# tuannv-github/srsRAN_Project

Hardware: AMD Instinct MI355X
Metric: PDSCH+PUSCH codeblocks/s @ 100 MHz 273-PRB 4x4 MIMO (PDSCH 4 layers, PUSCH 4 layers x 4 rx) (higher is better)
Workload: dtype int8+fp32; 1 GPU; BASELINE metric (PDSCH+PUSCH codeblocks/s @ 100 MHz 273-PRB 4x4 MIMO): full PDSCH+PUSCH slot pipeline, 100 MHz numerology-1 273 PRB, 256QAM R=948/1024; parallelism=single GPU

## Files before the change

### srsran_project_amd/csrc/pdsch_modulator.hip

```cpp
#include <hip/hip_runtime.h>

#include "bf16_device.h"

#include "gold_sequence.h"
#include "pdsch_modulator_args.h"

#pragma clang fp contract(off)

namespace srs_amd {
namespace {

__device__ __forceinline__ float2 cmul_simd(float2 x, float wr, float wi)
{
  return make_float2(__builtin_fmaf(x.x, wr, -(x.y * wi)), __builtin_fmaf(x.y, wr, x.x * wi));
}

__device__ __forceinline__ uint32_t to_bf16(float f)
{
  uint32_t u = __float_as_uint(f);
  u += 0x7fffu + ((u >> 16) & 1u);
  return u >> 16;
}

__device__ __forceinline__ uint32_t pack_cbf16(float2 v)
{
  return cbf16_pack(v.x, v.y);
}

__device__ __forceinline__ float2 qam_point(uint32_t idx, int qm)
{
  float off = -1.0f, re = 0.0f, im = 0.0f;
  for (int j = 0; j < qm / 2; ++j) {
    re += off;
    im += off;
    off *= 2.0f;
    re = ((idx >> (2 * j + 1)) & 1u) ? re : -re;
    im = ((idx >> (2 * j)) & 1u) ? im : -im;
  }
  return make_float2(re, im);
}

__device__ __forceinline__ uint32_t data_re_before(const uint32_t* row, uint32_t nof_prb, uint32_t k)
{
  const uint32_t prb = k / PDSCH_NRE;
  if (prb >= nof_prb) {
    const uint32_t e = row[nof_prb - 1];
    return (e >> 12) + __builtin_popcount(e & 0xfffu);
  }
  const uint32_t e = row[prb];
  return (e >> 12) + __builtin_popcount(e & ((1u << (k % PDSCH_NRE)) - 1u));
}

__device__ __forceinline__ uint32_t codeword_word(const uint8_t* cw, uint32_t nof_bytes, uint32_t w)
{
  uint32_t v = 0;
#pragma unroll
  for (int q = 0; q < 4; ++q) {
    const uint32_t p = 4 * w + q;
    const uint32_t b = p < nof_bytes ? cw[p] : 0u;
    v |= (__builtin_bitreverse32(b) >> 24) << (8 * q);
  }
  return v;
}

constexpr int MAX_WORDS = PDSCH_THREADS + 2;

template <bool MULTI, typename T>
__device__ __forceinline__ const T& item_of(const T& own, const T* items)
{
  if constexpr (MULTI) {
    return items[blockIdx.z];
  } else {
    return own;
  }
}

template <bool MULTI>
__global__ __launch_bounds__(PDSCH_THREADS) void pdsch_map_kernel(pdsch_map_args own, const pdsch_map_args* items)
{
  const pdsch_map_args& a = item_of<MULTI>(own, items);
  if (MULTI && (blockIdx.x >= a.nof_tiles || blockIdx.y >= a.nof_symbols)) {
    return;
  }
  __shared__ uint32_t scrambled[MAX_WORDS];
  __shared__ float2   s_qam[256];

  const uint32_t  l   = a.first_symbol + blockIdx.y;
  const uint32_t  k0  = a.first_subc + blockIdx.x * PDSCH_THREADS;
  const uint32_t  k   = k0 + threadIdx.x;
  const uint32_t* row = a.re_table + l * a.nof_prb;
  const uint32_t  kend = min(k0 + PDSCH_THREADS, a.nof_subc);

  const uint32_t bits_per_re = static_cast<uint32_t>(a.nof_layers) * (a.qm < 2 ? 1u : static_cast<uint32_t>(a.qm));
  const uint32_t j_lo        = data_re_before(row, a.nof_prb, k0);
  const uint32_t j_hi        = data_re_before(row, a.nof_prb, kend);
  if (j_hi == j_lo) {
    return;
  }
  const uint32_t w_lo = j_lo * bits_per_re / 32;
  const uint32_t w_hi = (j_hi * bits_per_re + 31) / 32;

  const uint8_t* cw        = a.codewords + static_cast<uint64_t>(blockIdx.z) * a.cw_stride;
  const uint32_t nof_bytes = (a.nof_bits + 7) / 8;
  if (a.qm >= 2 && threadIdx.x < (1u << a.qm)) {
    s_qam[threadIdx.x] = qam_point(threadIdx.x, a.qm);
  }
  const uint32_t nw = w_hi - w_lo;
  for (uint32_t q = threadIdx.x; q < nw; q += PDSCH_THREADS) {
    scrambled[q] = codeword_word(cw, nof_bytes, w_lo + q) ^ a.scr[w_lo + q];
  }
  __syncthreads();

  if (k >= kend) {
    return;
  }
  const uint32_t e   = row[k / PDSCH_NRE];
  const uint32_t bit = k % PDSCH_NRE;
  if (((e >> bit) & 1u) == 0) {
    return;
  }
  const uint32_t j = (e >> 12) + __builtin_popcount(e & ((1u << bit) - 1u));
  if ((j + 1) * bits_per_re > a.nof_bits) {
    return;
  }

  const int bps = a.qm < 2 ? 1 : a.qm;
  float2    x[4];
#pragma unroll
  for (int v = 0; v < 4; ++v) {
    if (v < a.nof_layers) {
      const uint32_t s   = j * a.nof_layers + v;
      const uint32_t o   = s * bps - w_lo * 32;
      const uint64_t win = static_cast<uint64_t>(scrambled[o / 32]) |
                           (static_cast<uint64_t>(scrambled[min(o / 32 + 1, static_cast<uint32_t>(MAX_WORDS - 1))])
                            << 32);
      const uint32_t seq = static_cast<uint32_t>(win >> (o % 32)) & ((1u << bps) - 1u);
      const uint32_t idx = __builtin_bitreverse32(seq) >> (32 - bps);
      if (a.qm >= 2) {
        x[v] = s_qam[idx];
      } else {
        const float b = idx ? -1.0f : 1.0f;
        x[v]          = make_float2((a.qm == 0 && (s & 1u)) ? -b : b, b);
      }
    }
  }

  uint32_t* grid = a.grids + static_cast<uint64_t>(blockIdx.z) * a.grid_stride + l * a.nof_subc + k;
#pragma unroll
  for (int p = 0; p < 4; ++p) {
    if (p < a.nof_ports) {
      float2 y = cmul_simd(x[0], a.w[0][p][0], a.w[0][p][1]);
#pragma unroll
      for (int v = 1; v < 4; ++v) {
        if (v < a.nof_layers) {
          const float2 t = cmul_simd(x[v], a.w[v][p][0], a.w[v][p][1]);
          y.x            = y.x + t.x;
          y.y            = y.y + t.y;
        }
      }
      grid[static_cast<uint64_t>(p) * a.port_stride] = pack_cbf16(y);
    }
  }
}

constexpr int DMRS_THREADS      = 256;
constexpr int DMRS_GRIDS_PER_WG = 4;
constexpr int DMRS_MAX_WORDS    = 64;

template <bool MULTI>
__global__ __launch_bounds__(DMRS_THREADS) void dmrs_pdsch_kernel(dmrs_pdsch_args own, const dmrs_pdsch_args* items,
                                                                 uint32_t nof_grids)
{
  const dmrs_pdsch_args& a = item_of<MULTI>(own, items);
  __shared__ uint32_t    s_words[DMRS_MAX_WORDS];
  const uint32_t         e0 = blockIdx.x * DMRS_THREADS;
  if (e0 >= a.nof_crb * PDSCH_NRE || (MULTI && blockIdx.y >= a.nof_dmrs_symbols)) {
    return;
  }
  const int      nd = a.type2 ? 4 : 6;
  const uint32_t l  = a.symbol[blockIdx.y];
  const uint32_t i_lo   = e0 / PDSCH_NRE;
  const uint32_t i_hi   = min(a.nof_crb, (e0 + DMRS_THREADS + PDSCH_NRE - 1) / PDSCH_NRE) - 1;
  const uint32_t w_lo   = 2u * nd * (a.crbs[i_lo] - a.reference_point_k_rb) / 32;
  const uint32_t w_hi   = (2u * nd * (a.crbs[i_hi] - a.reference_point_k_rb) + 2u * nd - 1) / 32;
  const bool     shared = w_hi - w_lo < DMRS_MAX_WORDS;
  if (shared && threadIdx.x <= w_hi - w_lo) {
    uint32_t x1, x2;
    gold_state(a.jump, a.c_init[blockIdx.y], 32 * (w_lo + threadIdx.x), x1, x2);
    s_words[threadIdx.x] = gold_next32(x1, x2);
  }
  __syncthreads();
  const uint32_t e = e0 + threadIdx.x;
  const uint32_t i = e / PDSCH_NRE;
  const uint32_t r = e - i * PDSCH_NRE;
  if (i >= a.nof_crb) {
    return;
  }
  const uint32_t g = a.type2 ? (r % 6) / 2 : (r & 1u);
  const uint32_t t = a.type2 ? (r & 1u) + 2 * (r / 6) : (r >> 1);
  if (2 * static_cast<int>(g) >= a.nof_layers) {
    return;
  }
  const uint32_t crb = a.crbs[i];
  const uint32_t b   = 2u * nd * (crb - a.reference_point_k_rb) + 2 * t;
  uint32_t       word;
  if (shared) {
    word = s_words[b / 32 - w_lo];
  } else {
    uint32_t x1, x2;
    gold_state(a.jump, a.c_init[blockIdx.y], 32 * (b / 32), x1, x2);
    word = gold_next32(x1, x2);
  }
  const uint32_t bits = word >> (b % 32);
  const float    amp  = a.amplitude;
  const float2   base = make_float2((bits & 1u) ? -amp : amp, (bits & 2u) ? -amp : amp);
  const float2   seq1 = (t & 1u) ? make_float2(-base.x, -base.y) : base;
  const uint32_t sc   = crb * PDSCH_NRE + r;
  const uint32_t z0   = MULTI ? 0u : blockIdx.z * DMRS_GRIDS_PER_WG;
  const uint32_t z1   = MULTI ? 1u : min(nof_grids, z0 + DMRS_GRIDS_PER_WG);
  uint32_t       y[4];
#pragma unroll
  for (int p = 0; p < 4; ++p) {
    if (p < a.nof_ports) {
      float2 v = cmul_simd(base, a.w[2 * g][p][0], a.w[2 * g][p][1]);
      if (2 * static_cast<int>(g) + 1 < a.nof_layers) {
        const float2 u = cmul_simd(seq1, a.w[2 * g + 1][p][0], a.w[2 * g + 1][p][1]);
        v.x            = v.x + u.x;
        v.y            = v.y + u.y;
      }
      y[p] = pack_cbf16(v);
    }
  }
  for (uint32_t z = z0; z < z1; ++z) {
    uint32_t* grid = a.grids + static_cast<uint64_t>(MULTI ? blockIdx.z : z) * a.grid_stride +
                     l * (a.port_stride / 14) + sc;
#pragma unroll
    for (int p = 0; p < 4; ++p) {
      if (p < a.nof_ports) {
        grid[static_cast<uint64_t>(p) * a.port_stride] = y[p];
      }
    }
  }
}

}

hipError_t launch_pdsch_map(const pdsch_map_args& a, uint32_t nof_symbols, uint32_t span_subc, uint32_t nof_cws,
                            hipStream_t stream)
{
  if (nof_symbols == 0 || span_subc == 0 || nof_cws == 0) {
    return hipSuccess;
  }
  const dim3 grid((span_subc + PDSCH_THREADS - 1) / PDSCH_THREADS, nof_symbols, nof_cws);
  hipLaunchKernelGGL(pdsch_map_kernel<false>, grid, dim3(PDSCH_THREADS), 0, stream, a, nullptr);
  return hipGetLastError();
}

hipError_t launch_dmrs_pdsch(const dmrs_pdsch_args& a, uint32_t nof_grids, hipStream_t stream)
{
  if (a.nof_crb == 0 || a.nof_dmrs_symbols == 0 || nof_grids == 0) {
    return hipSuccess;
  }
  const dim3 grid((a.nof_crb * PDSCH_NRE + DMRS_THREADS - 1) / DMRS_THREADS, a.nof_dmrs_symbols,
                  (nof_grids + DMRS_GRIDS_PER_WG - 1) / DMRS_GRIDS_PER_WG);
  hipLaunchKernelGGL(dmrs_pdsch_kernel<false>, grid, dim3(DMRS_THREADS), 0, stream, a, nullptr, nof_grids);
  return hipGetLastError();
}

hipError_t launch_pdsch_map_items(const pdsch_map_args* items, uint32_t count, uint32_t max_tiles,
                                  uint32_t max_symbols, hipStream_t stream)
{
  if (count == 0 || max_tiles == 0 || max_symbols == 0) {
    return hipSuccess;
  }
  hipLaunchKernelGGL(pdsch_map_kernel<true>, dim3(max_tiles, max_symbols, count), dim3(PDSCH_THREADS), 0, stream,
                     pdsch_map_args{}, items);
  return hipGetLastError();
}

hipError_t launch_dmrs_pdsch_items(const dmrs_pdsch_args* items, uint32_t count, uint32_t max_crb_blocks,
                                   uint32_t max_symbols, hipStream_t stream)
{
  if (count == 0 || max_crb_blocks == 0 || max_symbols == 0) {
    return hipSuccess;
  }
  hipLaunchKernelGGL(dmrs_pdsch_kernel<true>, dim3(max_crb_blocks, max_symbols, count), dim3(DMRS_THREADS), 0,
                     stream, dmrs_pdsch_args{}, items, 1u);
  return hipGetLastError();
}

__global__ __launch_bounds__(64) void ptrs_pdsch_kernel(const ptrs_pdsch_args* items)
{
  const ptrs_pdsch_args& a = items[blockIdx.z];
  const uint32_t         i = blockIdx.x * 64 + threadIdx.x;
  const uint32_t         l = blockIdx.y;
  if (i >= a.nof_prb || ((a.symbol_mask >> l) & 1u) == 0) {
    return;
  }
  const uint32_t b    = a.bit0 + i * a.bit_step;
  const uint32_t bits = gold_word(a.jump, a.c_init, 32 * (b / 32)) >> (b % 32);
  const float2   x    = make_float2((bits & 1u) ? -a.amplitude : a.amplitude, (bits & 2u) ? -a.amplitude : a.amplitude);
  const uint32_t crb  = a.rb_begin + i * a.rb_stride;
  const float*   w    = a.w + 2 * (crb / a.prg_size) * a.nof_ports;
  uint32_t*      re   = a.grid + static_cast<uint64_t>(l) * a.nof_subc + crb * PDSCH_NRE + a.k;
  for (uint32_t p = 0; p < a.nof_ports; ++p) {
    re[static_cast<uint64_t>(p) * a.port_stride] = pack_cbf16(cmul_simd(x, w[2 * p], w[2 * p + 1]));
  }
}

hipError_t launch_ptrs_pdsch_items(const ptrs_pdsch_args* items, uint32_t count, uint32_t max_prb, hipStream_t stream)
{
  if (count == 0 || max_prb == 0) {
    return hipSuccess;
  }
  hipLaunchKernelGGL(ptrs_pdsch_kernel, dim3((max_prb + 63) / 64, PDSCH_NSYMB, count), dim3(64), 0, stream, items);
  return hipGetLastError();
}

}
```

### srsran_project_amd/csrc/pdsch_modulator_api.cpp

```cpp
#include "srsran_amd/pdsch_modulator.h"

#include <hip/hip_runtime.h>

#include "api_common.h"
#include "device_buffer.h"
#include "gold_sequence.h"
#include "modulation_args.h"
#include "pdsch_modulator_args.h"
#include "staged_call.h"
#include <algorithm>
#include <cmath>
#include <cstring>
#include <mutex>
#include <vector>

using namespace srs_amd;

struct srs_amd_pdsch_modulator {
  int           device = 0;
  hipStream_t   stream = nullptr;
  uint32_t*     d_jump = nullptr;
  device_buffer scratch;
  device_buffer slot_items;
  pinned_stage  stage;
  stream_order  order;
  std::mutex    mtx;
  ~srs_amd_pdsch_modulator()
  {
    (void)hipSetDevice(device);
    if (stream) {
      (void)hipStreamSynchronize(stream);
      (void)hipStreamDestroy(stream);
    }
    (void)hipFree(d_jump);
  }
};

struct srs_amd_pdsch_mod_plan {
  int            device = 0;
  pdsch_map_args args{};
  uint32_t       nof_symbols = 0;
  uint32_t       span_subc   = 0;
  uint32_t       nof_re      = 0;
  uint32_t*      d_table     = nullptr;
  uint32_t*      d_scr       = nullptr;
  ~srs_amd_pdsch_mod_plan()
  {
    (void)hipSetDevice(device);
    (void)hipFree(d_table);
    (void)hipFree(d_scr);
  }
};

namespace {

bool crb_bit(const uint8_t* mask, uint32_t i)
{
  return i < SRS_AMD_MAX_RB && ((mask[i / 8] >> (i % 8)) & 1u);
}

bool valid_qm(int qm)
{
  return qm == 0 || qm == 1 || qm == 2 || qm == 4 || qm == 6 || qm == 8;
}

float modulation_scaling(int qm)
{
  if (qm < 2) {
    return static_cast<float>(M_SQRT1_2);
  }
  const int L   = 1 << qm;
  float     sum = 0;
  for (int i = 0; i < L; ++i) {
    float off = -1, re = 0, im = 0;
    for (int j = 0; j < qm / 2; ++j) {
      re += off;
      im += off;
      off *= 2;
      re *= ((i & (1 << (2 * j + 1))) != 0) ? +1 : -1;
      im *= ((i & (1 << (2 * j + 0))) != 0) ? +1 : -1;
    }
    sum += re * re + im * im;
  }
  return std::sqrt(1 / (sum / static_cast<float>(L)));
}

uint32_t dmrs_prb_mask(uint32_t type, uint32_t nof_cdm_groups_without_data)
{
  uint32_t m = 0;
  for (uint32_t k = 0; k < 12; ++k) {
    const bool in = type == 1 ? (k % 2) < nof_cdm_groups_without_data : (k % 6) < 2 * nof_cdm_groups_without_data;
    m |= in ? (1u << k) : 0u;
  }
  return m;
}

int check_weights(uint32_t nof_layers, uint32_t nof_ports)
{
  if (nof_layers < 1 || nof_layers > SRS_AMD_MAX_LAYERS) {
    return fail(SRS_AMD_EINVAL, "The number of layers (i.e., %u) must be in range [1, %d].", nof_layers,
                SRS_AMD_MAX_LAYERS);
  }
  if (nof_ports < nof_layers || nof_ports > SRS_AMD_MAX_TX_PORTS) {
    return fail(SRS_AMD_EINVAL, "The number of antennas (i.e., %u) must be in range [%u, %d].", nof_ports,
                nof_layers, SRS_AMD_MAX_TX_PORTS);
  }
  return SRS_AMD_OK;
}

}

extern "C" {

int srs_amd_pdsch_modulator_create(srs_amd_pdsch_modulator** mod, int device)
{
  if (mod == nullptr) {
    return fail(SRS_AMD_EINVAL, "null handle pointer");
  }
  *mod   = nullptr;
  int rc = select_device(device);
  if (rc != SRS_AMD_OK) {
    return rc;
  }
  auto* m                 = new srs_amd_pdsch_modulator();
  m->device               = device;
  std::vector<uint32_t> j = gold_jump_tables();
  hipError_t            e = hipMalloc(&m->d_jump, j.size() * sizeof(uint32_t));
  if (e == hipSuccess) {
    e = hipMemcpy(m->d_jump, j.data(), j.size() * sizeof(uint32_t), hipMemcpyHostToDevice);
  }
  if (e == hipSuccess) {
    e = hipStreamCreateWithFlags(&m->stream, hipStreamNonBlocking);
  }
  if (e != hipSuccess) {
    delete m;
    return hip_fail(e, "PDSCH modulator tables");
  }
  *mod = m;
  return SRS_AMD_OK;
}

void srs_amd_pdsch_modulator_destroy(srs_amd_pdsch_modulator* mod)
{
  delete mod;
}

int srs_amd_pdsch_mod_plan_create(srs_amd_pdsch_modulator*        mod,
                                  const srs_amd_pdsch_mod_config* cfg,
                                  uint32_t                        nof_subc,
                                  srs_amd_pdsch_mod_plan**        plan,
                                  uint32_t*                       nof_re)
{
  if (mod == nullptr || cfg == nullptr || plan == nullptr) {
    return fail(SRS_AMD_EINVAL, "null argument");
  }
  *plan = nullptr;
  if (nof_subc == 0 || nof_subc % 12 != 0 || nof_subc > 12 * SRS_AMD_MAX_RB) {
    return fail(SRS_AMD_EINVAL, "Invalid number of grid subcarriers (i.e., %u).", nof_subc);
  }
  if (!valid_qm(cfg->modulation)) {
    return fail(SRS_AMD_EINVAL, "Invalid modulation scheme %d.", cfg->modulation);
  }
  int rc = check_weights(cfg->nof_layers, cfg->nof_ports);
  if (rc != SRS_AMD_OK) {
    return rc;
  }
  if (cfg->nof_symbols == 0 || cfg->start_symbol + cfg->nof_symbols > PDSCH_NSYMB) {
    return fail(SRS_AMD_EINVAL, "The time allocation of the transmission [%u, %u) exceeds the slot boundary.",
                cfg->start_symbol, cfg->start_symbol + cfg->nof_symbols);
  }
  if (cfg->dmrs_type != 1 && cfg->dmrs_type != 2) {
    return fail(SRS_AMD_EINVAL, "Invalid DM-RS type %u.", cfg->dmrs_type);
  }
  if (cfg->nof_cdm_groups_without_data < 1 || cfg->nof_cdm_groups_without_data > (cfg->dmrs_type == 1 ? 2u : 3u)) {
    return fail(SRS_AMD_EINVAL, "Invalid number of CDM groups without data (i.e., %u).",
                cfg->nof_cdm_groups_without_data);
  }
  if (cfg->nof_reserved > SRS_AMD_MAX_RE_PATTERNS) {
    return fail(SRS_AMD_EINVAL, "Too many reserved RE patterns (i.e., %u).", cfg->nof_reserved);
  }
  const uint32_t nof_prb = nof_subc / 12;
  uint32_t       lo = nof_prb, hi = 0;
// ... 1 lines not shown
    if (crb_bit(cfg->crb_mask, c)) {
      lo = std::min(lo, c);
      hi = c + 1;
    }
  }
  for (uint32_t c = nof_prb; c < SRS_AMD_MAX_RB; ++c) {
    if (crb_bit(cfg->crb_mask, c)) {
      return fail(SRS_AMD_EINVAL, "Allocated CRB %u exceeds the grid bandwidth (%u RB).", c, nof_prb);
    }
  }
  if (hi == 0) {
    return fail(SRS_AMD_EINVAL, "Empty frequency allocation.");
  }

  const uint32_t        dmrs_re = dmrs_prb_mask(cfg->dmrs_type, cfg->nof_cdm_groups_without_data);
  std::vector<uint32_t> table(PDSCH_NSYMB * nof_prb, 0);
  uint32_t              count = 0;
  for (uint32_t l = 0; l < PDSCH_NSYMB; ++l) {
    const bool in_time = l >= cfg->start_symbol && l < cfg->start_symbol + cfg->nof_symbols;
    for (uint32_t c = 0; c < nof_prb; ++c) {
      uint32_t m = (in_time && crb_bit(cfg->crb_mask, c)) ? 0xfffu : 0u;
      if (m != 0) {
        for (uint32_t r = 0; r < cfg->nof_reserved; ++r) {
          const srs_amd_re_pattern& p = cfg->reserved[r];
          if (((p.symbols >> l) & 1u) && crb_bit(p.crb_mask, c)) {
            m &= ~static_cast<uint32_t>(p.re_mask);
          }
        }
        if (((cfg->dmrs_symbol_mask >> l) & 1u) && c >= cfg->bwp_start && c < cfg->bwp_start + cfg->bwp_size) {
          m &= ~dmrs_re;
        }
      }
      table[l * nof_prb + c] = (count << 12) | m;
      count += static_cast<uint32_t>(__builtin_popcount(m));
    }
  }

  auto* p                 = new srs_amd_pdsch_mod_plan();
  p->device               = mod->device;
  p->nof_re               = count;
  p->nof_symbols          = cfg->nof_symbols;
  p->span_subc            = (hi - lo) * 12;
  pdsch_map_args& a       = p->args;
  a.jump                  = mod->d_jump;
  a.port_stride           = PDSCH_NSYMB * nof_subc;
  a.nof_subc              = nof_subc;
  a.nof_prb               = nof_prb;
  a.c_init                = (cfg->rnti << 15) + cfg->n_id;
  a.first_symbol          = cfg->start_symbol;
  a.qm                    = cfg->modulation;
  a.nof_layers            = static_cast<int32_t>(cfg->nof_layers);
  a.nof_ports             = static_cast<int32_t>(cfg->nof_ports);
  a.first_subc            = lo * 12;
  a.nof_symbols           = cfg->nof_symbols;
  a.nof_tiles             = (p->span_subc + PDSCH_THREADS - 1) / PDSCH_THREADS;
  float scaling           = modulation_scaling(cfg->modulation);
  if (std::isnormal(cfg->scaling)) {
    scaling *= cfg->scaling;
  }
  for (uint32_t v = 0; v < cfg->nof_layers; ++v) {
    for (uint32_t q = 0; q < cfg->nof_ports; ++q) {
      a.w[v][q][0] = cfg->weights[v][q][0] * scaling;
      a.w[v][q][1] = cfg->weights[v][q][1] * scaling;
    }
  }
  hipError_t e = hipSetDevice(mod->device);
  if (e == hipSuccess) {
    e = hipMalloc(&p->d_table, table.size() * sizeof(uint32_t));
  }
  if (e == hipSuccess) {
    e = hipMemcpy(p->d_table, table.data(), table.size() * sizeof(uint32_t), hipMemcpyHostToDevice);
  }
  const uint32_t bps       = cfg->modulation < 2 ? 1u : static_cast<uint32_t>(cfg->modulation);
  const uint32_t nof_words = (count * cfg->nof_layers * bps + 31) / 32 + 1;
  if (e == hipSuccess) {
    e = hipMalloc(&p->d_scr, nof_words * sizeof(uint32_t));
  }
  if (e == hipSuccess) {
    e = launch_gold_words(mod->d_jump, a.c_init, p->d_scr, nof_words, nullptr);
  }
  if (e == hipSuccess) {
    e = hipStreamSynchronize(nullptr);
  }
  if (e != hipSuccess) {
    delete p;
    return hip_fail(e, "PDSCH modulator plan");
  }
  a.scr      = p->d_scr;
  a.re_table = p->d_table;
  *plan      = p;
  if (nof_re != nullptr) {
    *nof_re = count;
  }
  return SRS_AMD_OK;
}

void srs_amd_pdsch_mod_plan_destroy(srs_amd_pdsch_mod_plan* plan)
{
  delete plan;
}

int srs_amd_pdsch_modulate_batch(srs_amd_pdsch_modulator*      mod,
                                 const srs_amd_pdsch_mod_plan* plan,
                                 uint32_t*                     d_grids,
                                 uint64_t                      grid_stride,
                                 const uint8_t*                d_codewords,
                                 uint32_t                      cw_stride,
                                 uint32_t                      nof_bits,
                                 uint32_t                      nof_cws,
                                 void*                         stream)
{
  if (mod == nullptr || plan == nullptr) {
    return fail(SRS_AMD_EINVAL, "null argument");
  }
  const pdsch_map_args& pa  = plan->args;
  const uint32_t        bps = pa.qm < 2 ? 1u : static_cast<uint32_t>(pa.qm);
  if (nof_bits == 0 || nof_bits % (pa.nof_layers * bps) != 0) {
    return fail(SRS_AMD_EINVAL, "The codeword length (i.e., %u bits) is not a whole number of REs (%d layers x %u bits).",
                nof_bits, pa.nof_layers, bps);
  }
  if (nof_cws == 0) {
    return SRS_AMD_OK;
  }
  if (d_grids == nullptr || d_codewords == nullptr) {
    return fail(SRS_AMD_EINVAL, "null device buffer");
  }
  if (nof_cws > 1 && (cw_stride < (nof_bits + 7) / 8 || grid_stride < static_cast<uint64_t>(pa.nof_ports) *
                                                                           pa.port_stride)) {
    return fail(SRS_AMD_EINVAL, "codeword or grid stride too small");
  }
  pdsch_map_args a = pa;
  a.codewords      = d_codewords;
  a.grids          = d_grids;
  a.grid_stride    = grid_stride;
  a.cw_stride      = cw_stride;
  a.nof_bits       = nof_bits;
  hipError_t e     = hipSetDevice(mod->device);
  if (e == hipSuccess) {
    e = launch_pdsch_map(a, plan->nof_symbols, plan->span_subc, nof_cws, static_cast<hipStream_t>(stream));
  }
  return e == hipSuccess ? SRS_AMD_OK : hip_fail(e, "pdsch_map_kernel launch");
}

int srs_amd_pdsch_modulate(srs_amd_pdsch_modulator*      mod,
                           const srs_amd_pdsch_mod_plan* plan,
                           uint32_t*                     grid,
                           uint32_t                      grid_ports,
                           const uint8_t*                codeword,
                           uint32_t                      nof_bits)
{
  if (mod == nullptr || plan == nullptr || grid == nullptr || codeword == nullptr) {
    return fail(SRS_AMD_EINVAL, "null argument");
  }
  if (grid_ports < static_cast<uint32_t>(plan->args.nof_ports)) {
    return fail(SRS_AMD_EINVAL, "The precoding number of ports (i.e., %d) exceeds the grid number of ports (i.e., %u).",
                plan->args.nof_ports, grid_ports);
  }
  std::lock_guard<std::mutex> lock(mod->mtx);
  const size_t                grid_bytes = static_cast<size_t>(grid_ports) * plan->args.port_stride * 4;
  const size_t                cw_bytes   = (nof_bits + 7) / 8;
  hipError_t                  e          = hipSetDevice(mod->device);
  if (e == hipSuccess) {
    e = mod->scratch.ensure(grid_bytes + align_up(cw_bytes, 256) + 256);
  }
  if (e != hipSuccess) {
    return hip_fail(e, "PDSCH modulator scratch");
  }
  auto* d_grid = mod->scratch.as<uint32_t>();
  auto* d_cw   = mod->scratch.as<uint8_t>() + align_up(grid_bytes, 256);
  e            = hipMemcpyAsync(d_grid, grid, grid_bytes, hipMemcpyHostToDevice, mod->stream);
  if (e == hipSuccess) {
    e = hipMemcpyAsync(d_cw, codeword, cw_bytes, hipMemcpyHostToDevice, mod->stream);
  }
  if (e != hipSuccess) {
    return hip_fail(e, "PDSCH modulator upload");
  }
  int rc = srs_amd_pdsch_modulate_batch(mod, plan, d_grid, 0, d_cw, static_cast<uint32_t>(cw_bytes), nof_bits, 1,
                                        mod->stream);
  if (rc != SRS_AMD_OK) {
    (void)hipStreamSynchronize(mod->stream);
    return rc;
  }
  e = hipMemcpyAsync(grid, d_grid, grid_bytes, hipMemcpyDeviceToHost, mod->stream);
  if (e == hipSuccess) {
    e = hipStreamSynchronize(mod->stream);
  }
  return e == hipSuccess ? SRS_AMD_OK : hip_fail(e, "PDSCH modulator download");
}

}

struct ptrs_layout {
// ... 68 lines not shown
  ptrs_layout o;
  int         rc = ptrs_pattern(c, o);
  if (rc != SRS_AMD_OK) {
    return rc;
  }
  if (c->nof_ports == 0 || c->nof_ports > SRS_AMD_MAX_TX_PORTS || c->nof_prg == 0 || c->prg_size == 0 ||
      c->weights == nullptr) {
    return fail(SRS_AMD_EINVAL, "Invalid PT-RS precoding (%u ports, %u PRGs of %u PRBs).", c->nof_ports, c->nof_prg,
                c->prg_size);
  }
  if (o.rb_end > nof_subc / 12 || o.mask_begin < c->reference_point_k_rb) {
    return fail(SRS_AMD_EINVAL, "PT-RS CRBs outside the grid or below the reference point.");
  }
  const uint32_t nd = c->dmrs_type == 1 ? 6 : 4;
  a                 = ptrs_pdsch_args{};
  a.jump            = mod->d_jump;
  a.port_stride     = PDSCH_NSYMB * nof_subc;
  a.nof_subc        = nof_subc;
  a.rb_begin        = o.rb_begin;
  a.rb_stride       = o.stride;
  a.nof_prb         = o.rb_end > o.rb_begin ? (o.rb_end - o.rb_begin + o.stride - 1) / o.stride : 0;
  if (a.nof_prb != 0 && (o.rb_begin + (a.nof_prb - 1) * o.stride) / c->prg_size >= c->nof_prg) {
    return fail(SRS_AMD_EINVAL, "PT-RS CRBs beyond the precoding PRGs.");
  }
  a.k           = o.k;
  a.symbol_mask = o.symbol_mask;
  const uint32_t l0    = c->dmrs_symbols_mask != 0 ? static_cast<uint32_t>(__builtin_ctz(c->dmrs_symbols_mask)) : 0u;
  const uint32_t nid   = c->scrambling_id;
  const uint32_t nscid = c->n_scid ? 1u : 0u;
  a.c_init   = ((PDSCH_NSYMB * c->slot_index + l0 + 1) * (2 * nid + 1) * (1u << 17) + (2 * nid + nscid)) % (1u << 31);
  a.bit0     = 2 * ((o.rb_begin - c->reference_point_k_rb) * nd + o.k / 2);
  a.bit_step = 2 * nd * o.stride;
  a.amplitude = static_cast<float>(M_SQRT1_2 * c->amplitude);
  a.nof_ports = c->nof_ports;
  a.prg_size  = c->prg_size;
  return SRS_AMD_OK;
}

static int make_dmrs_args(const srs_amd_pdsch_modulator* mod, const srs_amd_dmrs_pdsch_config* cfg, uint32_t nof_subc,
                          dmrs_pdsch_args& a)
{
  int rc = check_weights(cfg->nof_layers, cfg->nof_ports);
  if (rc != SRS_AMD_OK) {
    return rc;
  }
  if (cfg->type != 1 && cfg->type != 2) {
    return fail(SRS_AMD_EINVAL, "Invalid DM-RS type %u.", cfg->type);
  }
  if (nof_subc == 0 || nof_subc % 12 != 0 || nof_subc > 12 * SRS_AMD_MAX_RB) {
    return fail(SRS_AMD_EINVAL, "Invalid number of grid subcarriers (i.e., %u).", nof_subc);
  }
  a = dmrs_pdsch_args{};
  a.jump                 = mod->d_jump;
  a.port_stride          = PDSCH_NSYMB * nof_subc;
  a.reference_point_k_rb = cfg->reference_point_k_rb;
  a.type2                = cfg->type == 2 ? 1 : 0;
  a.nof_layers           = static_cast<int32_t>(cfg->nof_layers);
  a.nof_ports            = static_cast<int32_t>(cfg->nof_ports);
  a.amplitude            = static_cast<float>(M_SQRT1_2 * cfg->amplitude);
  for (uint32_t c = 0; c < SRS_AMD_MAX_RB; ++c) {
    if (crb_bit(cfg->crb_mask, c)) {
      if (c >= nof_subc / 12) {
        return fail(SRS_AMD_EINVAL, "DM-RS CRB %u exceeds the grid bandwidth.", c);
      }
      if (c < cfg->reference_point_k_rb) {
        return fail(SRS_AMD_EINVAL, "DM-RS CRB %u below the reference point %u.", c, cfg->reference_point_k_rb);
      }
      a.crbs[a.nof_crb++] = static_cast<uint16_t>(c);
    }
  }
  const unsigned nslot = cfg->slot_index;
  const unsigned nid   = cfg->scrambling_id;
  const unsigned nscid = cfg->n_scid ? 1 : 0;
  for (uint32_t l = 0; l < PDSCH_NSYMB; ++l) {
    if ((cfg->symbols_mask >> l) & 1u) {
      const uint32_t i = a.nof_dmrs_symbols++;
      a.symbol[i]      = static_cast<uint8_t>(l);
      a.lprime[i]      = (l > 0 && ((cfg->symbols_mask >> (l - 1)) & 1u)) ? 1 : 0;
      a.c_init[i] = ((PDSCH_NSYMB * nslot + l + 1) * (2 * nid + 1) * (1u << 17) + (2 * nid + nscid)) % (1u << 31);
    }
  }
  for (uint32_t v = 0; v < cfg->nof_layers; ++v) {
    for (uint32_t q = 0; q < cfg->nof_ports; ++q) {
      a.w[v][q][0] = cfg->weights[v][q][0];
      a.w[v][q][1] = cfg->weights[v][q][1];
    }
  }
  return SRS_AMD_OK;
}

extern "C" {

int srs_amd_dmrs_pdsch_map_batch(srs_amd_pdsch_modulator*         mod,
                                 const srs_amd_dmrs_pdsch_config* cfg,
                                 uint32_t*                        d_grids,
                                 uint64_t                         grid_stride,
                                 uint32_t                         nof_subc,
                                 uint32_t                         nof_grids,
                                 void*                            stream)
{
  if (mod == nullptr || cfg == nullptr) {
    return fail(SRS_AMD_EINVAL, "null argument");
  }
  dmrs_pdsch_args a;
  int             rc = make_dmrs_args(mod, cfg, nof_subc, a);
  if (rc != SRS_AMD_OK) {
// ... 58 lines not shown
                                const srs_amd_pdsch_slot_pdu* pdus,
                                uint32_t                      nof_pdus,
                                uint32_t*                     d_grids,
                                uint64_t                      grid_stride,
                                uint32_t                      nof_grids,
                                uint32_t                      nof_subc,
                                const uint8_t*                d_codewords,
                                void*                         stream)
{
  if (mod == nullptr || (nof_pdus != 0 && pdus == nullptr)) {
    return fail(SRS_AMD_EINVAL, "null argument");
  }
  if (nof_pdus == 0) {
    return SRS_AMD_OK;
  }
  std::vector<pdsch_map_args>  maps;
  std::vector<dmrs_pdsch_args> dmrs;
  std::vector<ptrs_pdsch_args> ptrs;
  std::vector<float>           ptrs_w;
  std::vector<size_t>          ptrs_woff;
  uint32_t                     max_tiles = 0, max_symbols = 0, max_blocks = 0, max_dmrs_symbols = 0, max_ptrs = 0;
  for (uint32_t i = 0; i != nof_pdus; ++i) {
    const srs_amd_pdsch_slot_pdu& u = pdus[i];
    if (u.d_grid == nullptr && (d_grids == nullptr || u.grid >= nof_grids)) {
      return fail(SRS_AMD_EINVAL, "PDU %u: grid index %u out of range (or no grid).", i, u.grid);
    }
    const bool      own  = u.d_grid != nullptr;
    uint32_t* const grid = own ? u.d_grid : d_grids + u.grid * grid_stride;
    const uint32_t  ng   = own ? 1u : nof_grids;
    if (u.plan != nullptr) {
      const pdsch_map_args& pa  = u.plan->args;
      const uint32_t        bps = pa.qm < 2 ? 1u : static_cast<uint32_t>(pa.qm);
      if (pa.nof_subc != nof_subc) {
        return fail(SRS_AMD_EINVAL, "PDU %u: plan for %u subcarriers, grid of %u.", i, pa.nof_subc, nof_subc);
      }
      if (u.nof_bits == 0 || u.nof_bits % (pa.nof_layers * bps) != 0) {
        return fail(SRS_AMD_EINVAL, "PDU %u: the codeword length (i.e., %u bits) is not a whole number of REs.", i,
                    u.nof_bits);
      }
      if (ng > 1 && grid_stride < static_cast<uint64_t>(pa.nof_ports) * pa.port_stride) {
        return fail(SRS_AMD_EINVAL, "grid stride too small");
      }
      if (d_codewords == nullptr) {
        return fail(SRS_AMD_EINVAL, "null device buffer");
      }
      pdsch_map_args a = pa;
      a.codewords      = d_codewords + u.cw_offset;
      a.grids          = grid;
      a.grid_stride    = 0;
      a.cw_stride      = 0;
      a.nof_bits       = u.nof_bits;
      maps.push_back(a);
      max_tiles   = std::max(max_tiles, a.nof_tiles);
      max_symbols = std::max(max_symbols, a.nof_symbols);
    }
    if (u.dmrs != nullptr) {
      dmrs_pdsch_args a;
      int             rc = make_dmrs_args(mod, u.dmrs, nof_subc, a);
      if (rc != SRS_AMD_OK) {
        return rc;
      }
      if (ng > 1 && grid_stride < static_cast<uint64_t>(a.nof_ports) * a.port_stride) {
        return fail(SRS_AMD_EINVAL, "grid stride too small");
      }
      a.grids       = grid;
      a.grid_stride = 0;
      if (a.nof_crb != 0 && a.nof_dmrs_symbols != 0) {
        dmrs.push_back(a);
        max_blocks       = std::max(max_blocks, (a.nof_crb * PDSCH_NRE + 255) / 256);
        max_dmrs_symbols = std::max(max_dmrs_symbols, a.nof_dmrs_symbols);
      }
    }
    if (u.ptrs != nullptr) {
      ptrs_pdsch_args a;
      int             rc = make_ptrs_args(mod, u.ptrs, nof_subc, a);
      if (rc != SRS_AMD_OK) {
        return rc;
      }
      if (ng > 1 && grid_stride < static_cast<uint64_t>(a.nof_ports) * a.port_stride) {
        return fail(SRS_AMD_EINVAL, "grid stride too small");
      }
      a.grid = grid;
      if (a.nof_prb != 0 && a.symbol_mask != 0) {
        ptrs_woff.push_back(ptrs_w.size());
        ptrs_w.insert(ptrs_w.end(), u.ptrs->weights, u.ptrs->weights + 2 * u.ptrs->nof_prg * u.ptrs->nof_ports);
        ptrs.push_back(a);
        max_ptrs = std::max(max_ptrs, a.nof_prb);
      }
    }
  }
  const size_t o_dmrs = align_up(sizeof(pdsch_map_args) * maps.size(), 256);
  const size_t o_ptrs = align_up(o_dmrs + sizeof(dmrs_pdsch_args) * dmrs.size(), 256);
  const size_t o_w    = align_up(o_ptrs + sizeof(ptrs_pdsch_args) * ptrs.size(), 256);
  const size_t total  = ptrs.empty() ? o_dmrs + sizeof(dmrs_pdsch_args) * dmrs.size() : o_w + sizeof(float) * ptrs_w.size();
  if (total == 0) {
    return SRS_AMD_OK;
  }
  auto                        s = static_cast<hipStream_t>(stream);
  std::lock_guard<std::mutex> lock(mod->mtx);
  staged_call call("PDSCH modulator slot", mod->device, mod->slot_items, total, mod->stage, total, mod->order, s);
  if (!call.ok()) {
    return call.finish();
  }
  std::memcpy(call.host(), maps.data(), sizeof(pdsch_map_args) * maps.size());
  std::memcpy(call.host(o_dmrs), dmrs.data(), sizeof(dmrs_pdsch_args) * dmrs.size());
  auto* d = mod->slot_items.as<uint8_t>();
  for (size_t q = 0; q != ptrs.size(); ++q) {
// ... 44 lines not shown
```

### srsran_project_amd/csrc/pdsch_modulator_args.h

```cpp
#pragma once

#include <hip/hip_runtime.h>

#include <cstdint>

namespace srs_amd {

constexpr int PDSCH_NSYMB   = 14;
constexpr int PDSCH_NRE     = 12;
constexpr int PDSCH_MAX_RB  = 275;
constexpr int PDSCH_THREADS = 256;

struct pdsch_map_args {
  const uint8_t*  codewords;
  uint32_t*       grids;
  const uint32_t* re_table;
  const uint32_t* jump;
  const uint32_t* scr;
  uint64_t        grid_stride;
  uint32_t        port_stride;
  uint32_t        nof_subc;
  uint32_t        nof_prb;
  uint32_t        cw_stride;
  uint32_t        nof_bits;
  uint32_t        c_init;
  uint32_t        first_symbol;
  int32_t         qm;
  int32_t         nof_layers;
  int32_t         nof_ports;
  uint32_t        first_subc;
  uint32_t        nof_symbols;
  uint32_t        nof_tiles;
  float           w[4][4][2];
};

struct dmrs_pdsch_args {
  uint32_t*       grids;
  const uint32_t* jump;
  uint64_t        grid_stride;
  uint32_t        port_stride;
  uint32_t        nof_crb;
  uint32_t        reference_point_k_rb;
  int32_t         type2;
  int32_t         nof_layers;
  int32_t         nof_ports;
  float           amplitude;
  uint32_t        nof_dmrs_symbols;
  uint8_t         symbol[PDSCH_NSYMB];
  uint8_t         lprime[PDSCH_NSYMB];
  uint32_t        c_init[PDSCH_NSYMB];
  float           w[4][4][2];
  uint16_t        crbs[PDSCH_MAX_RB];
};

struct ptrs_pdsch_args {
  uint32_t*       grid;
  const uint32_t* jump;
  const float*    w;
  uint32_t        port_stride;
  uint32_t        nof_subc;
  uint32_t        c_init;
  uint32_t        bit0;
  uint32_t        bit_step;
  uint32_t        rb_begin;
  uint32_t        rb_stride;
  uint32_t        nof_prb;
  uint32_t        k;
  uint32_t        symbol_mask;
  float           amplitude;
  uint32_t        nof_ports;
  uint32_t        prg_size;
};

hipError_t launch_ptrs_pdsch_items(const ptrs_pdsch_args* items, uint32_t count, uint32_t max_prb, hipStream_t stream);

hipError_t launch_pdsch_map(const pdsch_map_args& a, uint32_t nof_symbols, uint32_t span_subc, uint32_t nof_cws,
                            hipStream_t stream);
hipError_t launch_dmrs_pdsch(const dmrs_pdsch_args& a, uint32_t nof_grids, hipStream_t stream);

hipError_t launch_pdsch_map_items(const pdsch_map_args* items, uint32_t count, uint32_t max_tiles,
                                  uint32_t max_symbols, hipStream_t stream);
hipError_t launch_dmrs_pdsch_items(const dmrs_pdsch_args* items, uint32_t count, uint32_t max_crb_blocks,
                                   uint32_t max_symbols, hipStream_t stream);

}
```

Measured before the change: 25.76 million codeblocks/s.

## Restructure PDSCH mapper: skip DMRS-only symbols, two symbols per workgroup, word codeword loads

```diff
diff --git a/srsran_project_amd/csrc/pdsch_modulator.hip b/srsran_project_amd/csrc/pdsch_modulator.hip
--- a/srsran_project_amd/csrc/pdsch_modulator.hip
+++ b/srsran_project_amd/csrc/pdsch_modulator.hip
@@ -27,43 +27,65 @@
   return cbf16_pack(v.x, v.y);
 }
 
-__device__ __forceinline__ float2 qam_point(uint32_t idx, int qm)
-{
-  float off = -1.0f, re = 0.0f, im = 0.0f;
-  for (int j = 0; j < qm / 2; ++j) {
-    re += off;
-    im += off;
-    off *= 2.0f;
-    re = ((idx >> (2 * j + 1)) & 1u) ? re : -re;
-    im = ((idx >> (2 * j)) & 1u) ? im : -im;
-  }
-  return make_float2(re, im);
-}
-
-__device__ __forceinline__ uint32_t data_re_before(const uint32_t* row, uint32_t nof_prb, uint32_t k)
-{
-  const uint32_t prb = k / PDSCH_NRE;
-  if (prb >= nof_prb) {
-    const uint32_t e = row[nof_prb - 1];
-    return (e >> 12) + __builtin_popcount(e & 0xfffu);
-  }
-  const uint32_t e = row[prb];
-  return (e >> 12) + __builtin_popcount(e & ((1u << (k % PDSCH_NRE)) - 1u));
-}
-
-__device__ __forceinline__ uint32_t codeword_word(const uint8_t* cw, uint32_t nof_bytes, uint32_t w)
-{
-  uint32_t v = 0;
-#pragma unroll
-  for (int q = 0; q < 4; ++q) {
-    const uint32_t p = 4 * w + q;
-    const uint32_t b = p < nof_bytes ? cw[p] : 0u;
-    v |= (__builtin_bitreverse32(b) >> 24) << (8 * q);
-  }
-  return v;
+struct qam_tables {
+  float v[4 + 16 + 64 + 256][2];
+};
+constexpr int qam_offset(int qm)
+{
+  return qm == 2 ? 0 : qm == 4 ? 4 : qm == 6 ? 20 : 84;
+}
+constexpr qam_tables make_qam_tables()
+{
+  qam_tables t{};
+  for (int qm = 2; qm <= 8; qm += 2) {
+    for (unsigned idx = 0; idx < (1u << qm); ++idx) {
+      float off = -1.0f, re = 0.0f, im = 0.0f;
+      for (int j = 0; j < qm / 2; ++j) {
+        re += off;
+        im += off;
+        off *= 2.0f;
+        re = ((idx >> (2 * j + 1)) & 1u) ? re : -re;
+        im = ((idx >> (2 * j)) & 1u) ? im : -im;
+      }
+      t.v[qam_offset(qm) + idx][0] = re;
+      t.v[qam_offset(qm) + idx][1] = im;
+    }
+  }
+  return t;
+}
+__device__ const qam_tables QAM_POINTS = make_qam_tables();
+
+__device__ __forceinline__ uint32_t data_re_before(uint32_t e, uint32_t nof_prb, uint32_t k)
+{
+  const uint32_t below = k / PDSCH_NRE >= nof_prb ? 0xfffu : (1u << (k % PDSCH_NRE)) - 1u;
+  return (e >> 12) + __builtin_popcount(e & below);
+}
+
+struct cw_fetch {
+  uint32_t lo, hi;
+};
+__device__ __forceinline__ cw_fetch codeword_fetch(const uint8_t* cw, uint32_t nof_bytes, uint32_t w)
+{
+  const uint32_t m     = static_cast<uint32_t>(reinterpret_cast<uintptr_t>(cw) & 3u);
+  const uint8_t* first = cw - m;
+  const uint32_t last  = ((m + nof_bytes + 3u) & ~3u) - 4u;
+  cw_fetch       f;
+  f.lo = *reinterpret_cast<const uint32_t*>(first + min(4 * w, last));
+  f.hi = m != 0 ? *reinterpret_cast<const uint32_t*>(first + min(4 * w + 4, last)) : 0u;
+  return f;
+}
+__device__ __forceinline__ uint32_t codeword_word(const cw_fetch& f, const uint8_t* cw, uint32_t nof_bytes, uint32_t w)
+{
+  const uint32_t m    = static_cast<uint32_t>(reinterpret_cast<uintptr_t>(cw) & 3u);
+  const uint32_t n    = 4 * w < nof_bytes ? nof_bytes - 4 * w : 0u;
+  const uint32_t keep = n >= 4 ? 0xffffffffu : (1u << (8 * n)) - 1u;
+  const uint64_t both = static_cast<uint64_t>(f.lo) | (static_cast<uint64_t>(f.hi) << 32);
+  const uint32_t x    = static_cast<uint32_t>(both >> (8 * m)) & keep;
+  return __builtin_bswap32(__builtin_bitreverse32(x));
 }
 
 constexpr int MAX_WORDS = PDSCH_THREADS + 2;
+constexpr int SYMS_PER_WG = 2;
 
 template <bool MULTI, typename T>
 __device__ __forceinline__ const T& item_of(const T& own, const T* items)
@@ -75,77 +97,26 @@
   }
 }
 
-template <bool MULTI>
-__global__ __launch_bounds__(PDSCH_THREADS) void pdsch_map_kernel(pdsch_map_args own, const pdsch_map_args* items)
-{
-  const pdsch_map_args& a = item_of<MULTI>(own, items);
-  if (MULTI && (blockIdx.x >= a.nof_tiles || blockIdx.y >= a.nof_symbols)) {
-    return;
-  }
-  __shared__ uint32_t scrambled[MAX_WORDS];
-  __shared__ float2   s_qam[256];
-
-  const uint32_t  l   = a.first_symbol + blockIdx.y;
-  const uint32_t  k0  = a.first_subc + blockIdx.x * PDSCH_THREADS;
-  const uint32_t  k   = k0 + threadIdx.x;
-  const uint32_t* row = a.re_table + l * a.nof_prb;
-  const uint32_t  kend = min(k0 + PDSCH_THREADS, a.nof_subc);
-
-  const uint32_t bits_per_re = static_cast<uint32_t>(a.nof_layers) * (a.qm < 2 ? 1u : static_cast<uint32_t>(a.qm));
-  const uint32_t j_lo        = data_re_before(row, a.nof_prb, k0);
-  const uint32_t j_hi        = data_re_before(row, a.nof_prb, kend);
-  if (j_hi == j_lo) {
-    return;
-  }
-  const uint32_t w_lo = j_lo * bits_per_re / 32;
-  const uint32_t w_hi = (j_hi * bits_per_re + 31) / 32;
-
-  const uint8_t* cw        = a.codewords + static_cast<uint64_t>(blockIdx.z) * a.cw_stride;
-  const uint32_t nof_bytes = (a.nof_bits + 7) / 8;
-  if (a.qm >= 2 && threadIdx.x < (1u << a.qm)) {
-    s_qam[threadIdx.x] = qam_point(threadIdx.x, a.qm);
-  }
-  const uint32_t nw = w_hi - w_lo;
-  for (uint32_t q = threadIdx.x; q < nw; q += PDSCH_THREADS) {
-    scrambled[q] = codeword_word(cw, nof_bytes, w_lo + q) ^ a.scr[w_lo + q];
-  }
-  __syncthreads();
-
-  if (k >= kend) {
-    return;
-  }
-  const uint32_t e   = row[k / PDSCH_NRE];
-  const uint32_t bit = k % PDSCH_NRE;
-  if (((e >> bit) & 1u) == 0) {
-    return;
-  }
-  const uint32_t j = (e >> 12) + __builtin_popcount(e & ((1u << bit) - 1u));
-  if ((j + 1) * bits_per_re > a.nof_bits) {
-    return;
-  }
-
-  const int bps = a.qm < 2 ? 1 : a.qm;
-  float2    x[4];
+template <bool QAM>
+__device__ __forceinline__ void map_re(const pdsch_map_args& a, const float2* s_qam, uint32_t bits, uint32_t j,
+                                       uint32_t* grid)
+{
+  const int      bps = QAM ? a.qm : 1;
+  const uint32_t rev = __builtin_bitreverse32(bits);
+  float2         x[4];
 #pragma unroll
   for (int v = 0; v < 4; ++v) {
     if (v < a.nof_layers) {
-      const uint32_t s   = j * a.nof_layers + v;
-      const uint32_t o   = s * bps - w_lo * 32;
-      const uint64_t win = static_cast<uint64_t>(scrambled[o / 32]) |
-                           (static_cast<uint64_t>(scrambled[min(o / 32 + 1, static_cast<uint32_t>(MAX_WORDS - 1))])
-                            << 32);
-      const uint32_t seq = static_cast<uint32_t>(win >> (o % 32)) & ((1u << bps) - 1u);
-      const uint32_t idx = __builtin_bitreverse32(seq) >> (32 - bps);
-      if (a.qm >= 2) {
+      const uint32_t idx = (rev >> (32 - (v + 1) * bps)) & ((1u << bps) - 1u);
+      if constexpr (QAM) {
         x[v] = s_qam[idx];
       } else {
-        const float b = idx ? -1.0f : 1.0f;
-        x[v]          = make_float2((a.qm == 0 && (s & 1u)) ? -b : b, b);
-      }
-    }
-  }
-
-  uint32_t* grid = a.grids + static_cast<uint64_t>(blockIdx.z) * a.grid_stride + l * a.nof_subc + k;
+        const uint32_t s = j * a.nof_layers + v;
+        const float    b = idx ? -1.0f : 1.0f;
+        x[v]             = make_float2((a.qm == 0 && (s & 1u)) ? -b : b, b);
+      }
+    }
+  }
 #pragma unroll
   for (int p = 0; p < 4; ++p) {
     if (p < a.nof_ports) {
@@ -163,9 +134,127 @@
   }
 }
 
+template <bool MULTI>
+__global__ __launch_bounds__(PDSCH_THREADS) void pdsch_map_kernel(pdsch_map_args                     own,
+                                                                  const pdsch_map_args* __restrict__ items)
+{
+  const pdsch_map_args& a  = item_of<MULTI>(own, items);
+  const uint32_t        g0 = blockIdx.y * SYMS_PER_WG;
+  if (MULTI && (blockIdx.x >= a.nof_tiles || g0 >= a.nof_data_symbols)) {
+    return;
+  }
+  __shared__ uint32_t scrambled[SYMS_PER_WG][MAX_WORDS];
+  __shared__ float2   s_qam[256];
+
+  const uint32_t k0       = a.first_subc + blockIdx.x * PDSCH_THREADS;
+  const uint32_t k        = k0 + threadIdx.x;
+  const uint32_t kend     = min(k0 + PDSCH_THREADS, a.nof_subc);
+  const uint32_t last_prb = a.nof_prb - 1;
+
+  uint32_t l[SYMS_PER_WG], e[SYMS_PER_WG], e_lo[SYMS_PER_WG], e_hi[SYMS_PER_WG];
+#pragma unroll
+  for (int g = 0; g < SYMS_PER_WG; ++g) {
+    const uint32_t gi   = min(g0 + g, a.nof_data_symbols - 1);
+    l[g]                = static_cast<uint32_t>(a.data_symbols >> (4 * gi)) & 15u;
+    const uint32_t* row = a.re_table + l[g] * a.nof_prb;
+    e_lo[g]             = row[min(k0 / PDSCH_NRE, last_prb)];
+    e_hi[g]             = row[min(kend / PDSCH_NRE, last_prb)];
+    e[g]                = row[min(k / PDSCH_NRE, last_prb)];
+  }
+
+  const uint32_t bits_per_re = static_cast<uint32_t>(a.nof_layers) * (a.qm < 2 ? 1u : static_cast<uint32_t>(a.qm));
+  uint32_t       w_lo[SYMS_PER_WG], nw[SYMS_PER_WG];
+  uint32_t       any = 0;
+#pragma unroll
+  for (int g = 0; g < SYMS_PER_WG; ++g) {
+    const uint32_t j_lo = data_re_before(e_lo[g], a.nof_prb, k0);
+    const uint32_t j_hi = data_re_before(e_hi[g], a.nof_prb, kend);
+    const bool     live = g0 + g < a.nof_data_symbols && j_hi != j_lo;
+    w_lo[g]             = j_lo * bits_per_re / 32;
+    nw[g]               = live ? (j_hi * bits_per_re + 31) / 32 - w_lo[g] : 0u;
+    any |= nw[g];
+  }
+  if (any == 0) {
+    return;
+  }
+
+  const uint8_t* cw        = a.codewords + static_cast<uint64_t>(blockIdx.z) * a.cw_stride;
+  const uint32_t nof_bytes = (a.nof_bits + 7) / 8;
+  const bool     qam       = a.qm >= 2 && threadIdx.x < (1u << a.qm);
+  float2         point     = make_float2(0.0f, 0.0f);
+  if (qam) {
+    const float* p = QAM_POINTS.v[qam_offset(a.qm) + threadIdx.x];
+    point          = make_float2(p[0], p[1]);
+  }
+  const bool extra = threadIdx.x < MAX_WORDS - PDSCH_THREADS;
+  cw_fetch   f[SYMS_PER_WG], fx[SYMS_PER_WG];
+  uint32_t   c[SYMS_PER_WG], wi[SYMS_PER_WG], cx[SYMS_PER_WG], wx[SYMS_PER_WG];
+#pragma unroll
+  for (int g = 0; g < SYMS_PER_WG; ++g) {
+    const uint32_t last = max(nw[g], 1u) - 1u;
+    wi[g]               = w_lo[g] + min(threadIdx.x, last);
+    wx[g]               = w_lo[g] + min(threadIdx.x + PDSCH_THREADS, last);
+    f[g]                = codeword_fetch(cw, nof_bytes, wi[g]);
+    c[g]                = a.scr[wi[g]];
+    fx[g]               = cw_fetch{0u, 0u};
+    cx[g]               = 0;
+    if (extra) {
+      fx[g] = codeword_fetch(cw, nof_bytes, wx[g]);
+      cx[g] = a.scr[wx[g]];
+    }
+  }
+  if (qam) {
+    s_qam[threadIdx.x] = point;
+  }
+#pragma unroll
+  for (int g = 0; g < SYMS_PER_WG; ++g) {
+    if (threadIdx.x < nw[g]) {
+      scrambled[g][threadIdx.x] = codeword_word(f[g], cw, nof_bytes, wi[g]) ^ c[g];
+    }
+    if (extra && threadIdx.x + PDSCH_THREADS < nw[g]) {
+      scrambled[g][threadIdx.x + PDSCH_THREADS] = codeword_word(fx[g], cw, nof_bytes, wx[g]) ^ cx[g];
+    }
+  }
+  __syncthreads();
+
+  if (k >= kend) {
+    return;
+  }
+  const uint32_t bit = k % PDSCH_NRE;
+#pragma unroll
+  for (int g = 0; g < SYMS_PER_WG; ++g) {
+    if (nw[g] == 0 || ((e[g] >> bit) & 1u) == 0) {
+      continue;
+    }
+    const uint32_t j = (e[g] >> 12) + __builtin_popcount(e[g] & ((1u << bit) - 1u));
+    if ((j + 1) * bits_per_re > a.nof_bits) {
+      continue;
+    }
+    const uint32_t o    = j * bits_per_re - w_lo[g] * 32;
+    const uint64_t win  = static_cast<uint64_t>(scrambled[g][o / 32]) | (static_cast<uint64_t>(scrambled[g][o / 32 + 1]) << 32);
+    const uint32_t bits = static_cast<uint32_t>(win >> (o % 32));
+    uint32_t*      grid = a.grids + static_cast<uint64_t>(blockIdx.z) * a.grid_stride + l[g] * a.nof_subc + k;
+    if (a.qm >= 2) {
+      map_re<true>(a, s_qam, bits, j, grid);
+    } else {
+      map_re<false>(a, s_qam, bits, j, grid);
+    }
+  }
+}
+
 constexpr int DMRS_THREADS      = 256;
 constexpr int DMRS_GRIDS_PER_WG = 4;
 constexpr int DMRS_MAX_WORDS    = 64;
+
+__device__ __forceinline__ uint32_t dmrs_word(const dmrs_pdsch_args& a, uint32_t c_init, uint32_t w)
+{
+  if (w < GOLD_BASIS_WORDS) {
+    return gold_basis_word(a.gold_basis, c_init, w);
+  }
+  uint32_t x1, x2;
+  gold_state(a.jump, c_init, 32 * w, x1, x2);
+  return gold_next32(x1, x2);
+}
 
 template <bool MULTI>
 __global__ __launch_bounds__(DMRS_THREADS) void dmrs_pdsch_kernel(dmrs_pdsch_args own, const dmrs_pdsch_args* items,
@@ -185,9 +274,7 @@
   const uint32_t w_hi   = (2u * nd * (a.crbs[i_hi] - a.reference_point_k_rb) + 2u * nd - 1) / 32;
   const bool     shared = w_hi - w_lo < DMRS_MAX_WORDS;
   if (shared && threadIdx.x <= w_hi - w_lo) {
-    uint32_t x1, x2;
-    gold_state(a.jump, a.c_init[blockIdx.y], 32 * (w_lo + threadIdx.x), x1, x2);
-    s_words[threadIdx.x] = gold_next32(x1, x2);
+    s_words[threadIdx.x] = dmrs_word(a, a.c_init[blockIdx.y], w_lo + threadIdx.x);
   }
   __syncthreads();
   const uint32_t e = e0 + threadIdx.x;
@@ -203,14 +290,7 @@
   }
   const uint32_t crb = a.crbs[i];
   const uint32_t b   = 2u * nd * (crb - a.reference_point_k_rb) + 2 * t;
-  uint32_t       word;
-  if (shared) {
-    word = s_words[b / 32 - w_lo];
-  } else {
-    uint32_t x1, x2;
-    gold_state(a.jump, a.c_init[blockIdx.y], 32 * (b / 32), x1, x2);
-    word = gold_next32(x1, x2);
-  }
+  const uint32_t word = shared ? s_words[b / 32 - w_lo] : dmrs_word(a, a.c_init[blockIdx.y], b / 32);
   const uint32_t bits = word >> (b % 32);
   const float    amp  = a.amplitude;
   const float2   base = make_float2((bits & 1u) ? -amp : amp, (bits & 2u) ? -amp : amp);
@@ -245,13 +325,12 @@
 
 }
 
-hipError_t launch_pdsch_map(const pdsch_map_args& a, uint32_t nof_symbols, uint32_t span_subc, uint32_t nof_cws,
-                            hipStream_t stream)
-{
-  if (nof_symbols == 0 || span_subc == 0 || nof_cws == 0) {
-    return hipSuccess;
-  }
-  const dim3 grid((span_subc + PDSCH_THREADS - 1) / PDSCH_THREADS, nof_symbols, nof_cws);
+hipError_t launch_pdsch_map(const pdsch_map_args& a, uint32_t nof_cws, hipStream_t stream)
+{
+  if (a.nof_data_symbols == 0 || a.nof_tiles == 0 || nof_cws == 0) {
+    return hipSuccess;
+  }
+  const dim3 grid(a.nof_tiles, (a.nof_data_symbols + SYMS_PER_WG - 1) / SYMS_PER_WG, nof_cws);
   hipLaunchKernelGGL(pdsch_map_kernel<false>, grid, dim3(PDSCH_THREADS), 0, stream, a, nullptr);
   return hipGetLastError();
 }
@@ -268,13 +347,13 @@
 }
 
 hipError_t launch_pdsch_map_items(const pdsch_map_args* items, uint32_t count, uint32_t max_tiles,
-                                  uint32_t max_symbols, hipStream_t stream)
-{
-  if (count == 0 || max_tiles == 0 || max_symbols == 0) {
-    return hipSuccess;
-  }
-  hipLaunchKernelGGL(pdsch_map_kernel<true>, dim3(max_tiles, max_symbols, count), dim3(PDSCH_THREADS), 0, stream,
-                     pdsch_map_args{}, items);
+                                  uint32_t max_data_symbols, hipStream_t stream)
+{
+  if (count == 0 || max_tiles == 0 || max_data_symbols == 0) {
+    return hipSuccess;
+  }
+  const dim3 grid(max_tiles, (max_data_symbols + SYMS_PER_WG - 1) / SYMS_PER_WG, count);
+  hipLaunchKernelGGL(pdsch_map_kernel<true>, grid, dim3(PDSCH_THREADS), 0, stream, pdsch_map_args{}, items);
   return hipGetLastError();
 }
 
diff --git a/srsran_project_amd/csrc/pdsch_modulator_api.cpp b/srsran_project_amd/csrc/pdsch_modulator_api.cpp
--- a/srsran_project_amd/csrc/pdsch_modulator_api.cpp
+++ b/srsran_project_amd/csrc/pdsch_modulator_api.cpp
@@ -19,7 +19,8 @@
 struct srs_amd_pdsch_modulator {
   int           device = 0;
   hipStream_t   stream = nullptr;
-  uint32_t*     d_jump = nullptr;
+  uint32_t*     d_jump  = nullptr;
+  uint32_t*     d_basis = nullptr;
   device_buffer scratch;
   device_buffer slot_items;
   pinned_stage  stage;
@@ -33,6 +34,7 @@
       (void)hipStreamDestroy(stream);
     }
     (void)hipFree(d_jump);
+    (void)hipFree(d_basis);
   }
 };
 
@@ -128,6 +130,13 @@
   hipError_t            e = hipMalloc(&m->d_jump, j.size() * sizeof(uint32_t));
   if (e == hipSuccess) {
     e = hipMemcpy(m->d_jump, j.data(), j.size() * sizeof(uint32_t), hipMemcpyHostToDevice);
+  }
+  const std::vector<uint32_t> b = gold_word_basis();
+  if (e == hipSuccess) {
+    e = hipMalloc(&m->d_basis, b.size() * sizeof(uint32_t));
+  }
+  if (e == hipSuccess) {
+    e = hipMemcpy(m->d_basis, b.data(), b.size() * sizeof(uint32_t), hipMemcpyHostToDevice);
   }
   if (e == hipSuccess) {
     e = hipStreamCreateWithFlags(&m->stream, hipStreamNonBlocking);
@@ -235,8 +244,13 @@
   a.nof_layers            = static_cast<int32_t>(cfg->nof_layers);
   a.nof_ports             = static_cast<int32_t>(cfg->nof_ports);
   a.first_subc            = lo * 12;
-  a.nof_symbols           = cfg->nof_symbols;
   a.nof_tiles             = (p->span_subc + PDSCH_THREADS - 1) / PDSCH_THREADS;
+  for (uint32_t l = cfg->start_symbol; l < cfg->start_symbol + cfg->nof_symbols; ++l) {
+    const uint32_t* row = table.data() + l * nof_prb;
+    if (std::any_of(row, row + nof_prb, [](uint32_t e) { return (e & 0xfffu) != 0; })) {
+      a.data_symbols |= static_cast<uint64_t>(l) << (4 * a.nof_data_symbols++);
+    }
+  }
   float scaling           = modulation_scaling(cfg->modulation);
   if (std::isnormal(cfg->scaling)) {
     scaling *= cfg->scaling;
@@ -320,7 +334,7 @@
   a.nof_bits       = nof_bits;
   hipError_t e     = hipSetDevice(mod->device);
   if (e == hipSuccess) {
-    e = launch_pdsch_map(a, plan->nof_symbols, plan->span_subc, nof_cws, static_cast<hipStream_t>(stream));
+    e = launch_pdsch_map(a, nof_cws, static_cast<hipStream_t>(stream));
   }
   return e == hipSuccess ? SRS_AMD_OK : hip_fail(e, "pdsch_map_kernel launch");
 }
@@ -495,6 +509,7 @@
   }
   a = dmrs_pdsch_args{};
   a.jump                 = mod->d_jump;
+  a.gold_basis           = mod->d_basis;
   a.port_stride          = PDSCH_NSYMB * nof_subc;
   a.reference_point_k_rb = cfg->reference_point_k_rb;
   a.type2                = cfg->type == 2 ? 1 : 0;
@@ -659,7 +674,7 @@
       a.nof_bits       = u.nof_bits;
       maps.push_back(a);
       max_tiles   = std::max(max_tiles, a.nof_tiles);
-      max_symbols = std::max(max_symbols, a.nof_symbols);
+      max_symbols = std::max(max_symbols, a.nof_data_symbols);
     }
     if (u.dmrs != nullptr) {
       dmrs_pdsch_args a;
diff --git a/srsran_project_amd/csrc/pdsch_modulator_args.h b/srsran_project_amd/csrc/pdsch_modulator_args.h
--- a/srsran_project_amd/csrc/pdsch_modulator_args.h
+++ b/srsran_project_amd/csrc/pdsch_modulator_args.h
@@ -29,14 +29,16 @@
   int32_t         nof_layers;
   int32_t         nof_ports;
   uint32_t        first_subc;
-  uint32_t        nof_symbols;
   uint32_t        nof_tiles;
+  uint32_t        nof_data_symbols;
+  uint64_t        data_symbols;
   float           w[4][4][2];
 };
 
 struct dmrs_pdsch_args {
   uint32_t*       grids;
   const uint32_t* jump;
+  const uint32_t* gold_basis;
   uint64_t        grid_stride;
   uint32_t        port_stride;
   uint32_t        nof_crb;
@@ -74,12 +76,11 @@
 
 hipError_t launch_ptrs_pdsch_items(const ptrs_pdsch_args* items, uint32_t count, uint32_t max_prb, hipStream_t stream);
 
-hipError_t launch_pdsch_map(const pdsch_map_args& a, uint32_t nof_symbols, uint32_t span_subc, uint32_t nof_cws,
-                            hipStream_t stream);
+hipError_t launch_pdsch_map(const pdsch_map_args& a, uint32_t nof_cws, hipStream_t stream);
 hipError_t launch_dmrs_pdsch(const dmrs_pdsch_args& a, uint32_t nof_grids, hipStream_t stream);
 
 hipError_t launch_pdsch_map_items(const pdsch_map_args* items, uint32_t count, uint32_t max_tiles,
-                                  uint32_t max_symbols, hipStream_t stream);
+                                  uint32_t max_data_symbols, hipStream_t stream);
 hipError_t launch_dmrs_pdsch_items(const dmrs_pdsch_args* items, uint32_t count, uint32_t max_crb_blocks,
                                    uint32_t max_symbols, hipStream_t stream);
 
```

After: 25.96 million codeblocks/s (median of 6 runs). Within noise of the previous version (+0.8%).
